# ishika28/Beyond-Binary-Fake-User-Detection-A-Credibility-Aware-Graph-based-Recommender-System

Measured on NVIDIA B200. Metric: edges/sec (3-layer cred-weighted LightGCN fwd+bwd), higher is better.
Workload: dtype f32

## Files before the change

### beyond-binary-fake-user-detection-a-credibility-aware-graph-based-recommender-system_b200/_lib.py

```python
from __future__ import annotations

import ctypes as C
import os
import pathlib
import subprocess

import torch

PKG_DIR = pathlib.Path(__file__).resolve().parent
LIB_PATH = PKG_DIR / "libcredgcn.so"
CSRC_DIR = PKG_DIR / "csrc"

VARIANTS = {"cu": 0, "v2": 1, "da": 2}
ORDERS = {"jacobi": 0, "gs": 1}
PRECISIONS = {"fp32": 0, "bf16x3": 1, "bf16": 2}
OPTIONS = {"L2_TABLE_BYTES": 0, "SPARSE_FIRST_ADJOINT": 1, "PDL": 2, "P2P_ONESHOT_MAX": 3, "P2P_TIMING": 4,
           "P2P_TIMEOUT_MS": 5, "EVAL_DEBUG": 6, "HOT_ROWS": 7, "EVAL_GROUPS": 8}
LONG_ROW = 256
CHUNK = 256


class CgxError(RuntimeError):
    pass

# ... 24 lines not shown
    "cgx_graph_build_workspace_bytes": (C.c_size_t, [C.c_int64, C.c_int32, C.c_int32]),
    "cgx_graph_build": (C.c_int, [_P, _P, C.c_int64, C.c_int32, C.c_int32, _P, C.c_int, _P, _P, _P, _P, _P, _P,
                                  _P, _P, _P, _P, _P, _P, _P, _P, _P, C.c_int, _P, C.c_size_t, _P]),
    "cgx_user_csr": (C.c_int, [_P, _P, C.c_int64, C.c_int32, C.c_int32, _P, _P, _P, C.c_size_t, _P]),
    "cgx_row_schedule_workspace_bytes": (C.c_size_t, [C.c_int32]),
    "cgx_row_schedule": (C.c_int, [_P, C.c_int32, _P, C.POINTER(C.c_int32), C.POINTER(C.c_int32),
                                   C.POINTER(C.c_int32), _P, C.c_size_t, _P]),
    "cgx_row_schedule_chunks": (C.c_int, [C.c_int32, C.c_int32, C.c_int32, _P, _P, _P, C.c_size_t, _P]),
    "cgx_row_schedule_work": (C.c_int, [_P, _P, C.c_int32, C.c_int32, C.c_int32, _P, _P, _P, _P]),
    "cgx_spmm_workspace_bytes": (C.c_size_t, [_CSR, C.c_int32]),
    "cgx_spmm": (C.c_int, [_CSR, C.c_int, C.c_int32, _P, _P, _P, _P, C.c_float, _P, C.c_size_t, _P]),
    "cgx_spmm_sparse_rows": (C.c_int, [_CSR, C.c_int, C.c_int32, _P, _P, _P, _P, _P, C.c_float, _P, C.c_size_t, _P]),
    "cgx_row_flags": (C.c_int, [_P, C.c_int64, C.c_int32, _P, _P]),
    "cgx_spmm_ex": (C.c_int, [_CSR, C.c_int, C.c_int32, _P, _P, _P, _P, _P, _P, C.c_float, _P, C.c_size_t, _P]),
    "cgx_spmm_set_l2_table_bytes": (C.c_int64, [C.c_int64]),
    "cgx_propagate_workspace_bytes": (C.c_size_t, [_CSR, _CSR, C.c_int32]),
    "cgx_propagate_workspace_bytes_for": (C.c_size_t, [_CSR, _CSR, C.c_int32, C.c_int]),
    "cgx_propagate_fwd": (C.c_int, [_CSR, _CSR, C.c_int, C.c_int32, C.c_int32, _P, _P, _P, _P, _P,
                                    C.c_size_t, _P]),
    "cgx_propagate_bwd": (C.c_int, [_CSR, _CSR, C.c_int, C.c_int32, C.c_int32, _P, _P, _P, _P, _P,
                                    C.c_size_t, _P]),
    "cgx_propagate_bwd_flagged": (C.c_int, [_CSR, _CSR, C.c_int, C.c_int32, C.c_int32, _P, _P, _P, _P, _P, _P, _P,
                                            C.c_size_t, _P]),
    "cgx_bpr_mark_rows": (C.c_int, [_P, C.c_int64, C.c_int32, _P, _P, _P]),
    "cgx_bpr_clear_rows": (C.c_int, [_P, C.c_int64, C.c_int32, C.c_int32, _P, _P, _P, _P, _P]),
    "cgx_bpr_workspace_bytes": (C.c_size_t, [C.c_int64, C.c_int32, C.c_int32]),
    "cgx_bpr_plan_workspace_bytes": (C.c_size_t, [C.c_int64]),
    "cgx_bpr_plan": (C.c_int, [_P, _P, _P, C.c_int64, C.c_int32, C.c_int32, _P, _P, C.c_size_t, _P]),
    "cgx_bpr_fwd_bwd": (C.c_int, [_P, _P, _P, C.c_int64, C.c_int64, _P, C.c_int32, C.c_int32, C.c_int32, _P, _P, _P,
                                  _P, _P,
                                  C.c_float, C.c_float, _P, _P, _P, _P, _P, _P, C.c_size_t, _P]),
    "cgx_bpr_apply_ego": (C.c_int, [_P, _P, C.c_int64, C.c_int32, C.c_int32, _P, _P, _P, _P, _P]),
    "cgx_sampler_build_workspace_bytes": (C.c_size_t, [C.c_int32]),
    "cgx_sampler_build": (C.c_int, [_P, C.c_int32, C.c_double, _P, _P, _P, _P, _P, _P, C.c_size_t, _P]),
    "cgx_sample_triples": (C.c_int, [_P, C.c_int64, _P, _P, C.c_int32, _P, _P, _P, _P, _P, C.c_float,
                                     C.c_int32, C.c_uint64, C.c_uint64, _P, _P, _P, _P]),
    "cgx_tick": (C.c_int, [_P, _P]),
    "cgx_adam_step": (C.c_int, [_P, _P, _P, _P, C.c_int64, _P, _P, _P, _P, C.c_int64, C.c_float, C.c_float,
                                C.c_float, C.c_float, _P, C.c_int64, _P]),
    "cgx_comm_alloc": (C.c_int, [C.c_size_t, C.POINTER(C.c_void_p)]),
    "cgx_comm_free": (C.c_int, [_P]),
    "cgx_comm_ipc_handle": (C.c_int, [_P, _P]),
    "cgx_comm_ipc_open": (C.c_int, [_P, C.POINTER(C.c_void_p)]),
    "cgx_comm_ipc_close": (C.c_int, [_P]),
    "cgx_comm_allreduce": (C.c_int, [C.c_int, C.c_int, C.POINTER(C.c_void_p), C.c_size_t, C.c_size_t, C.c_size_t,
                                     C.c_int64, _P, _P]),
# ... 88 lines not shown
```

### beyond-binary-fake-user-detection-a-credibility-aware-graph-based-recommender-system_b200/csrc/spmm.cu

```cuda
#include "common.cuh"

namespace cgx {

constexpr int SP_THREADS = 256;

__device__ __forceinline__ void fma4(float4& a, float v, const float4& x) {
  a.x = fmaf(v, x.x, a.x);
  a.y = fmaf(v, x.y, a.y);
  a.z = fmaf(v, x.z, a.z);
  a.w = fmaf(v, x.w, a.w);
}
__device__ __forceinline__ float4 add4(const float4& a, const float4& b) {
  return make_float4(a.x + b.x, a.y + b.y, a.z + b.z, a.w + b.w);
}
__device__ __forceinline__ float4 scale4(const float4& a, float s) {
  return make_float4(a.x * s, a.y * s, a.z * s, a.w * s);
}

enum { POL_NORMAL = 0, POL_FIRST = 1, POL_LAST = 2 };
template <int POL>
__device__ __forceinline__ void ld256(const float4* p, float4& a, float4& b) {
  if (POL == POL_LAST) {
    asm volatile("ld.global.nc.L1::no_allocate.L2::evict_last.v8.f32 {%0,%1,%2,%3,%4,%5,%6,%7}, [%8];"
                 : "=f"(a.x), "=f"(a.y), "=f"(a.z), "=f"(a.w), "=f"(b.x), "=f"(b.y), "=f"(b.z), "=f"(b.w)
// ... 164 lines not shown
    if constexpr (V == 2) st256<POL>(ACC_OUT + o, a[0], a[1]);
    else {
#pragma unroll
      for (int v = 0; v < V; ++v) ACC_OUT[o + v] = a[v];
    }
  }
}

struct SpmmSched {
  const int32_t* perm;
  const int32_t* chunk_ptr;
  int32_t* arrive;
  int32_t n_chunks, n_huge;
};

template <int G, int V, int UNR, int MINB, bool NZ, bool PUSH, bool HOT>
__global__ void __launch_bounds__(SP_THREADS, MINB) k_spmm(const int32_t* __restrict__ idx,
                                                           const float* __restrict__ val, int64_t n_items,
                                                           SpmmSched sc, const float4* __restrict__ X,
                                                           float4* __restrict__ Y, const float4* ACC_IN,
                                                           float4* ACC_OUT, float acc_scale, float4* partial,
                                                           const uint8_t* __restrict__ nz,
                                                           const uint8_t* __restrict__ acc_nz,
                                                           const int4* __restrict__ work, const SpmmPush ps_in) {
  const SpmmPush ps = PUSH ? ps_in : SpmmPush{0ull, 0, 0};
  constexpr int ROW4 = G * V;
  asm volatile("griddepcontrol.launch_dependents;");
  const int lane = threadIdx.x & (G - 1);
  const uint32_t item = (blockIdx.x * uint32_t(SP_THREADS) + threadIdx.x) / G;
  const unsigned mask = group_mask<G>();
  float4 acc[V];
#pragma unroll
  for (int v = 0; v < V; ++v) acc[v] = make_float4(0.f, 0.f, 0.f, 0.f);
  if (item >= n_items) return;
  const int4 wd = __ldg(work + item);
  const int64_t begin = (int64_t(wd.y) << 32) | uint32_t(wd.x);
  idx += begin;
  val += begin;
  int32_t cf = 0;
  float wf = 0.f;
  if (lane < wd.z) {
    cf = ld_idx<HOT>(idx + lane);
    wf = ld_val<HOT>(val + lane);
  }
  asm volatile("griddepcontrol.wait;" ::: "memory");
  gather_batches<G, V, UNR, NZ, HOT>(idx, val, wd.z, X, lane, mask, cf, wf, acc, nz);
  if (item >= sc.n_chunks) {
    epilogue<G, V, HOT>(wd.w, lane, acc, Y, ACC_IN, ACC_OUT, acc_scale, acc_nz, ps);
    return;
  }
  const int32_t k = wd.w;
#pragma unroll
  for (int v = 0; v < V; ++v) __stcg(partial + int64_t(item) * ROW4 + lane * V + v, acc[v]);
  if (k < sc.n_huge) return;
  const int32_t c0 = __ldg(sc.chunk_ptr + k), c1 = __ldg(sc.chunk_ptr + k + 1);
  __threadfence();
  __syncwarp(mask);
  int prev = 0;
  if (lane == 0) prev = atomicAdd(sc.arrive + k, 1);
  prev = __shfl_sync(mask, prev, 0, G);
  if (prev != c1 - c0 - 1) return;
  __threadfence();
#pragma unroll
  for (int v = 0; v < V; ++v) acc[v] = make_float4(0.f, 0.f, 0.f, 0.f);
  for (int c = c0; c < c1; ++c) {
#pragma unroll
    for (int v = 0; v < V; ++v) acc[v] = add4(acc[v], __ldcg(partial + int64_t(c) * ROW4 + lane * V + v));
  }
  epilogue<G, V, HOT>(int64_t(__ldg(sc.perm + k)), lane, acc, Y, ACC_IN, ACC_OUT, acc_scale, acc_nz, ps);
  if (lane == 0) sc.arrive[k] = 0;
}

template <int G, int V>
__global__ void __launch_bounds__(SP_THREADS) k_spmm_finish(SpmmSched sc, const float4* __restrict__ partial,
                                                            float4* __restrict__ Y, const float4* ACC_IN,
                                                            float4* ACC_OUT, float acc_scale,
                                                            const uint8_t* __restrict__ acc_nz, const SpmmPush ps) {
  constexpr int GROUPS = SP_THREADS / G;
  constexpr int ROW4 = G * V;
  __shared__ float4 red[GROUPS][ROW4];
  const int k = blockIdx.x;
  const int lane = threadIdx.x & (G - 1), grp = threadIdx.x / G;
  const int c0 = __ldg(sc.chunk_ptr + k), c1 = __ldg(sc.chunk_ptr + k + 1);
  float4 acc[V];
#pragma unroll
  for (int v = 0; v < V; ++v) acc[v] = make_float4(0.f, 0.f, 0.f, 0.f);
  for (int c = c0 + grp; c < c1; c += GROUPS) {
#pragma unroll
    for (int v = 0; v < V; ++v) acc[v] = add4(acc[v], __ldg(partial + int64_t(c) * ROW4 + lane * V + v));
  }
#pragma unroll
  for (int v = 0; v < V; ++v) red[grp][lane * V + v] = acc[v];
  __syncthreads();
  if (grp == 0) {
#pragma unroll
    for (int v = 0; v < V; ++v) {
      float4 s = red[0][lane * V + v];
      for (int g = 1; g < GROUPS; ++g) s = add4(s, red[g][lane * V + v]);
      acc[v] = s;
    }
    epilogue<G, V, false>(int64_t(__ldg(sc.perm + k)), lane, acc, Y, ACC_IN, ACC_OUT, acc_scale, acc_nz, ps);
  }
}

// ... 1 lines not shown
  int64_t p = int64_t(blockIdx.x) * blockDim.x + threadIdx.x;
  if (p < n4) out[p] = scale4(in[p], s);
}

__global__ void k_row_flags(const uint4* __restrict__ X, int64_t n4, int32_t row4, uint8_t* __restrict__ flags) {
  const int64_t p = int64_t(blockIdx.x) * blockDim.x + threadIdx.x;
  if (p >= n4) return;
  const uint4 v = X[p];
  if ((v.x | v.y | v.z | v.w) & 0x7fffffffu) flags[p / row4] = 1;
}

static int row_flags(const float* X, int64_t n_rows, int32_t d, uint8_t* flags, cudaStream_t stream) {
  CGX_CUDA(cudaMemsetAsync(flags, 0, size_t(n_rows), stream));
  const int64_t n4 = n_rows * d / 4;
  if (n4 == 0) return CGX_OK;
  k_row_flags<<<(unsigned)ceil_div(n4, 256), 256, 0, stream>>>(reinterpret_cast<const uint4*>(X), n4, d / 4, flags);
  CGX_LAUNCH_CHECK();
  return CGX_OK;
}

template <int G, int V, int UNR, int MINB, bool NZ, bool PUSH, bool HOT>
static int launch_spmm(const cgx_csr* m, const float* val, const float* X, float* Y, const float* ACC_IN,
                       float* ACC_OUT, float acc_scale, void* workspace, size_t workspace_bytes,
                       cudaStream_t stream, const uint8_t* nz, const uint8_t* acc_nz, const SpmmPush ps) {
  constexpr int GROUPS = SP_THREADS / G;
  float4* partial = nullptr;
  if (m->n_long > 0) {
    size_t need = size_t(m->n_chunks) * G * V * sizeof(float4);
    CGX_REQUIRE(workspace != nullptr && workspace_bytes >= need, CGX_ERR_WORKSPACE,
                "spmm: workspace too small for %d long-row chunks", m->n_chunks);
    partial = static_cast<float4*>(workspace);
  }
  SpmmSched sc{m->perm, m->chunk_ptr, m->arrive, m->n_chunks, m->n_huge};
  const int64_t items = int64_t(m->n_chunks) + (m->n_rows - m->n_long);
  cudaLaunchConfig_t cfg = {};
  cfg.gridDim = dim3((unsigned)ceil_div(items, GROUPS));
  cfg.blockDim = dim3(SP_THREADS);
  cfg.dynamicSmemBytes = 0;
  cfg.stream = stream;
  cudaLaunchAttribute attr[1];
  attr[0].id = cudaLaunchAttributeProgrammaticStreamSerialization;
  attr[0].val.programmaticStreamSerializationAllowed = option(CGX_OPT_PDL) != 0 ? 1 : 0;
  cfg.attrs = attr;
  cfg.numAttrs = 1;
  CGX_CUDA(cudaLaunchKernelEx(&cfg, k_spmm<G, V, UNR, MINB, NZ, PUSH, HOT>, HOT ? m->idx_hint : m->idx, val, items, sc,
                              reinterpret_cast<const float4*>(X), reinterpret_cast<float4*>(Y),
                              reinterpret_cast<const float4*>(ACC_IN), reinterpret_cast<float4*>(ACC_OUT), acc_scale,
                              partial, nz, acc_nz, static_cast<const int4*>(m->work), ps));
  CGX_LAUNCH_CHECK();
  if (m->n_huge > 0) {
    k_spmm_finish<G, V><<<(unsigned)m->n_huge, SP_THREADS, 0, stream>>>(
        sc, partial, reinterpret_cast<float4*>(Y), reinterpret_cast<const float4*>(ACC_IN),
        reinterpret_cast<float4*>(ACC_OUT), acc_scale, acc_nz, ps);
    CGX_LAUNCH_CHECK();
  }
  return CGX_OK;
}

#define CGX_SPMM_ARGS m, val, X, Y, ACC_IN, ACC_OUT, acc_scale, ws, ws_bytes, stream, nz, acc_nz, ps

template <int G, int V, int UNR>
static int spmm_flavour(const cgx_csr* m, const float* val, const float* X, float* Y, const float* ACC_IN,
                        float* ACC_OUT, float acc_scale, void* ws, size_t ws_bytes, cudaStream_t stream,
                        const uint8_t* nz, const uint8_t* acc_nz, const SpmmPush ps, bool hot) {
  const bool push = ps.rows_per > 0;
  if constexpr (V == 2) {
    if (hot && nz == nullptr) {
      if (push) return launch_spmm<G, V, UNR, 4, false, true, true>(CGX_SPMM_ARGS);
      return launch_spmm<G, V, UNR, 4, false, false, true>(CGX_SPMM_ARGS);
    }
  }
  if (push) {
    if (nz) return launch_spmm<G, V, UNR, 4, true, true, false>(CGX_SPMM_ARGS);
    return launch_spmm<G, V, UNR, 4, false, true, false>(CGX_SPMM_ARGS);
  }
  if (nz) return launch_spmm<G, V, UNR, 4, true, false, false>(CGX_SPMM_ARGS);
  return launch_spmm<G, V, UNR, 4, false, false, false>(CGX_SPMM_ARGS);
}

#define CGX_FLAVOUR_ARGS m, val, X, Y, ACC_IN, ACC_OUT, acc_scale, ws, ws_bytes, stream, nz, acc_nz, ps, hot

static int spmm_dispatch(const cgx_csr* m, int use_bwd, int32_t d, const float* X, float* Y, const float* ACC_IN,
                         float* ACC_OUT, float acc_scale, void* ws, size_t ws_bytes, cudaStream_t stream,
                         const uint8_t* nz = nullptr, const SpmmPush ps = SpmmPush{0ull, 0, 0},
                         const uint8_t* acc_nz = nullptr) {
  CGX_REQUIRE(m && m->perm && m->work && (m->nnz == 0 || (m->idx && m->val_fwd && m->val_bwd)) && X, CGX_ERR_ARG,
              "spmm: NULL pointer (cgx_csr needs idx, both value arrays and the cgx_row_schedule* outputs)");
  CGX_REQUIRE(m->n_long == 0 || (m->chunk_ptr && m->arrive), CGX_ERR_ARG, "spmm: chunk tables missing");
  CGX_REQUIRE(Y || ACC_OUT || ps.rows_per > 0, CGX_ERR_ARG, "spmm: no output requested");
  const float* val = use_bwd ? m->val_bwd : m->val_fwd;
  if (m->n_rows == 0) return CGX_OK;
  const bool beyond_l2 = int64_t(m->n_cols) * int64_t(d) * 4 > option(CGX_OPT_L2_TABLE_BYTES);
  const bool hot = beyond_l2 && m->idx_hint != nullptr && option(CGX_OPT_HOT_ROWS) != 0;
  switch (d) {
    case 16: return spmm_flavour<4, 1, 4>(CGX_FLAVOUR_ARGS);
    case 32: return spmm_flavour<8, 1, 8>(CGX_FLAVOUR_ARGS);
    case 64:
      if (beyond_l2) return spmm_flavour<8, 2, 4>(CGX_FLAVOUR_ARGS);
      return spmm_flavour<16, 1, 8>(CGX_FLAVOUR_ARGS);
    case 128:
      if (beyond_l2) return spmm_flavour<16, 2, 4>(CGX_FLAVOUR_ARGS);
      return spmm_flavour<32, 1, 8>(CGX_FLAVOUR_ARGS);
    case 256: return spmm_flavour<32, 2, 4>(CGX_FLAVOUR_ARGS);
    default:
      set_error("spmm: emb_dim %d unsupported (16, 32, 64, 128, 256)", d);
      return CGX_ERR_UNSUPPORTED;
  }
}

__global__ void k_hot_flags(const int32_t* __restrict__ col_by_degree, int32_t n_hot, uint8_t* __restrict__ hot) {
  const int32_t k = blockIdx.x * blockDim.x + threadIdx.x;
  if (k < n_hot) hot[__ldg(col_by_degree + k)] = 1;
// ... 68 lines not shown

extern "C" int cgx_spmm_set_push_peers(void* const* peer_bases, int world) {
  CGX_REQUIRE(peer_bases != nullptr && world >= 1 && world <= 16, CGX_ERR_ARG, "spmm_set_push_peers: bad argument");
  char* h[16] = {nullptr};
  for (int p = 0; p < world; ++p) h[p] = static_cast<char*>(peer_bases[p]);
  CGX_CUDA(cudaMemcpyToSymbol(c_push_base, h, sizeof(h)));
  return CGX_OK;
}

extern "C" int cgx_spmm_push(const cgx_csr* m, int use_bwd_values, int32_t d, const float* X,
                             const uint8_t* x_row_nonzero, size_t stage_off, int rank, int world, int32_t rows_per,
                             void* workspace, size_t workspace_bytes, void* stream) {
  CGX_REQUIRE(m != nullptr && world >= 1 && world <= 16 && rank >= 0 && rank < world && rows_per > 0 &&
                  int64_t(rows_per) * world >= m->n_rows && stage_off % 16 == 0,
              CGX_ERR_ARG, "spmm_push: bad rank / world / rows_per");
  const SpmmPush ps{(unsigned long long)stage_off, rows_per, rank};
  return spmm_dispatch(m, use_bwd_values, d, X, nullptr, nullptr, nullptr, 1.0f, workspace, workspace_bytes,
                       static_cast<cudaStream_t>(stream), x_row_nonzero, ps);
}

extern "C" int cgx_row_flags(const float* X, int64_t n_rows, int32_t d, uint8_t* flags, void* stream) {
  CGX_REQUIRE(X && flags && n_rows >= 0 && d > 0 && d % 4 == 0, CGX_ERR_ARG, "row_flags: bad argument");
  return row_flags(X, n_rows, d, flags, static_cast<cudaStream_t>(stream));
}

static size_t propagate_ws(const cgx_csr* by_user, const cgx_csr* by_item, int32_t d, int n_buf) {
  if (!by_user || !by_item) return 0;
  size_t long_ws = spmm_ws(by_user, d) > spmm_ws(by_item, d) ? spmm_ws(by_user, d) : spmm_ws(by_item, d);
  return n_buf * (align_up(size_t(by_user->n_rows) * d * 4) + align_up(size_t(by_item->n_rows) * d * 4)) + long_ws +
         align_up(size_t(by_user->n_rows)) + align_up(size_t(by_item->n_rows)) + 256;
}

extern "C" size_t cgx_propagate_workspace_bytes(const cgx_csr* by_user, const cgx_csr* by_item, int32_t d) {
  return propagate_ws(by_user, by_item, d, 2);
}

extern "C" size_t cgx_propagate_workspace_bytes_for(const cgx_csr* by_user, const cgx_csr* by_item, int32_t d,
                                                    int order) {
  return propagate_ws(by_user, by_item, d, order == CGX_ORDER_GS ? 1 : 2);
}

extern "C" int cgx_propagate_fwd(const cgx_csr* by_user, const cgx_csr* by_item, int order, int32_t K, int32_t d,
                                 const float* e0_u, const float* e0_i, float* out_u, float* out_i,
                                 void* workspace, size_t workspace_bytes, void* stream_) {
  cudaStream_t stream = static_cast<cudaStream_t>(stream_);
  CGX_REQUIRE(by_user && by_item && e0_u && e0_i && out_u && out_i, CGX_ERR_ARG, "propagate_fwd: NULL pointer");
// ... 33 lines not shown
    ci = ni;
  }
  return CGX_OK;
}

__global__ void k_scale_rows(const float4* __restrict__ in, const uint8_t* __restrict__ nz, float4* __restrict__ out,
                             int64_t n_rows, int32_t row4, float s) {
  const int64_t r = (int64_t(blockIdx.x) * blockDim.x + threadIdx.x) / 32;
  if (r >= n_rows || __ldg(nz + r) == 0) return;
  for (int p = threadIdx.x & 31; p < row4; p += 32) out[r * row4 + p] = scale4(in[r * row4 + p], s);
}

extern "C" int cgx_propagate_bwd(const cgx_csr* by_user, const cgx_csr* by_item, int order, int32_t K, int32_t d,
                                 const float* g_u, const float* g_i, float* d_e0_u, float* d_e0_i,
                                 void* workspace, size_t workspace_bytes, void* stream_) {
  return cgx_propagate_bwd_flagged(by_user, by_item, order, K, d, g_u, g_i, nullptr, nullptr, d_e0_u, d_e0_i, workspace,
                                   workspace_bytes, stream_);
}

extern "C" int cgx_propagate_bwd_flagged(const cgx_csr* by_user, const cgx_csr* by_item, int order, int32_t K,
                                         int32_t d, const float* g_u, const float* g_i, const uint8_t* g_u_rows,
                                         const uint8_t* g_i_rows, float* d_e0_u, float* d_e0_i, void* workspace,
                                         size_t workspace_bytes, void* stream_) {
  cudaStream_t stream = static_cast<cudaStream_t>(stream_);
  CGX_REQUIRE((g_u_rows == nullptr) == (g_i_rows == nullptr), CGX_ERR_ARG,
              "propagate_bwd_flagged: pass both row-flag arrays or neither");
  CGX_REQUIRE(by_user && by_item && g_u && g_i && d_e0_u && d_e0_i, CGX_ERR_ARG, "propagate_bwd: NULL pointer");
  CGX_REQUIRE(K >= 1, CGX_ERR_ARG, "propagate_bwd: num_layers must be >= 1");
  CGX_REQUIRE(order == CGX_ORDER_JACOBI || order == CGX_ORDER_GS, CGX_ERR_ARG, "propagate_bwd: bad order");
  CGX_REQUIRE(workspace_bytes >= cgx_propagate_workspace_bytes_for(by_user, by_item, d, order), CGX_ERR_WORKSPACE,
              "propagate_bwd: workspace too small");
  const int64_t U = by_user->n_rows, I = by_item->n_rows;
  Arena ws(workspace, workspace_bytes);
  const bool one = order == CGX_ORDER_GS;
  float* ub[2];
  float* ib[2];
  ub[0] = ws.take<float>(U * d);
  ub[1] = one ? ub[0] : ws.take<float>(U * d);
  ib[0] = ws.take<float>(I * d);
  ib[1] = one ? ib[0] : ws.take<float>(I * d);
  size_t lws = spmm_ws(by_user, d) > spmm_ws(by_item, d) ? spmm_ws(by_user, d) : spmm_ws(by_item, d);
  void* lw = ws.take<char>(lws);
  CGX_REQUIRE(ws.ok, CGX_ERR_WORKSPACE, "propagate_bwd: workspace too small");
  const float s = 1.0f / float(K + 1);
  const bool given = g_u_rows != nullptr;
  const bool sparse = given || option(CGX_OPT_SPARSE_FIRST_ADJOINT) != 0;
  uint8_t* nz_u = given ? const_cast<uint8_t*>(g_u_rows) : ws.take<uint8_t>(U);
  uint8_t* nz_i = given ? const_cast<uint8_t*>(g_i_rows) : ws.take<uint8_t>(I);
  CGX_REQUIRE(ws.ok, CGX_ERR_WORKSPACE, "propagate_bwd: workspace too small");
  if (order == CGX_ORDER_JACOBI) {
    const float* bu = g_u;
    const float* bi = g_i;
    if (sparse && !given) {
      CGX_TRY(row_flags(g_u, U, d, nz_u, stream));
      CGX_TRY(row_flags(g_i, I, d, nz_i, stream));
    }
    for (int k = 0; k < K; ++k) {
      const bool last = k == K - 1;
      float* nu = last ? d_e0_u : ub[k & 1];
      float* ni = last ? d_e0_i : ib[k & 1];
      const float sc = last ? s : 1.0f;
      const bool sp = sparse && k == 0;
      const SpmmPush nops{0ull, 0, 0};
      CGX_TRY(spmm_dispatch(by_user, 1, d, bi, nullptr, g_u, nu, sc, lw, lws, stream, sp ? nz_i : nullptr, nops,
                            sparse ? nz_u : nullptr));
      CGX_TRY(spmm_dispatch(by_item, 1, d, bu, nullptr, g_i, ni, sc, lw, lws, stream, sp ? nz_u : nullptr, nops,
                            sparse ? nz_i : nullptr));
      bu = nu;
      bi = ni;
    }
  } else {
    const float* bu = g_u;
    if (sparse && !given) {
      CGX_TRY(row_flags(g_u, U, d, nz_u, stream));
      CGX_TRY(row_flags(g_i, I, d, nz_i, stream));
    }
    const SpmmPush nops{0ull, 0, 0};
    for (int k = 0; k < K; ++k) {
      const bool last = k == K - 1;
      float* ni = ib[0];
      float* nu = last ? d_e0_u : ub[k & 1];
      CGX_TRY(spmm_dispatch(by_item, 1, d, bu, nullptr, g_i, ni, 1.0f, lw, lws, stream,
                            sparse && k == 0 ? nz_u : nullptr, nops, sparse ? nz_i : nullptr));
      CGX_TRY(spmm_dispatch(by_user, 1, d, ni, nullptr, g_u, nu, last ? s : 1.0f, lw, lws, stream, nullptr, nops,
                            sparse ? nz_u : nullptr));
      bu = nu;
    }
    const int64_t n4 = I * d / 4;
    if (given) {
      CGX_CUDA(cudaMemsetAsync(d_e0_i, 0, size_t(I) * d * 4, stream));
      if (I > 0) {
        k_scale_rows<<<(unsigned)ceil_div(I * 32, 256), 256, 0, stream>>>(
            reinterpret_cast<const float4*>(g_i), nz_i, reinterpret_cast<float4*>(d_e0_i), I, d / 4, s);
        CGX_LAUNCH_CHECK();
      }
    } else {
      k_scale<<<(unsigned)ceil_div(n4, 256), 256, 0, stream>>>(reinterpret_cast<const float4*>(g_i),
                                                               reinterpret_cast<float4*>(d_e0_i), n4, s);
      CGX_LAUNCH_CHECK();
    }
  }
  return CGX_OK;
}
```

### beyond-binary-fake-user-detection-a-credibility-aware-graph-based-recommender-system_b200/model.py

```python
from __future__ import annotations

import torch

from . import _lib
from ._lib import check, lib, ptr, stream_ptr, workspace
from .graph import CredGraph, graph_of


def _f32c(t: torch.Tensor) -> torch.Tensor:
    if t.dtype != torch.float32:
        raise _lib.CgxError(f"credgcn kernels are fp32, got {t.dtype}")
    return t.contiguous()


def _i64c(t, device) -> torch.Tensor:
    return torch.as_tensor(t, device=device).to(torch.int64).contiguous()


def propagate_forward(graph: CredGraph, e0_u, e0_i, num_layers: int, order: str):
    e0_u, e0_i = _f32c(e0_u), _f32c(e0_i)
    d = e0_u.shape[1]
    out_u, out_i = torch.empty_like(e0_u), torch.empty_like(e0_i)
    ws = graph.propagate_workspace(d, order)
    with torch.cuda.device(graph.device):
# ... 37 lines not shown
def spmm_sparse_rows(csr, x, flags=None, use_bwd_values=False):
    x = _f32c(x)
    flags = row_flags(x) if flags is None else flags
    d = x.shape[1]
    y = torch.empty(csr.n_rows, d, dtype=torch.float32, device=x.device)
    ws = workspace(lib().cgx_spmm_workspace_bytes(csr.ref(), d), x.device)
    with torch.cuda.device(x.device):
        check(lib().cgx_spmm_sparse_rows(csr.ref(), int(use_bwd_values), d, ptr(x), ptr(flags), ptr(y), None, None,
                                         1.0, ptr(ws), ws.numel(), stream_ptr(x.device)))
    return y


def bpr_plan(graph: CredGraph, users, pos, neg, plan=None):
    dev = graph.device
    users, pos, neg = _i64c(users, dev), _i64c(pos, dev), _i64c(neg, dev)
    B = users.numel()
    if plan is None:
        plan = torch.empty(3 * B, dtype=torch.int64, device=dev)
    ws = workspace(lib().cgx_bpr_plan_workspace_bytes(B), dev)
    with torch.cuda.device(dev):
        check(lib().cgx_bpr_plan(ptr(users), ptr(pos), ptr(neg), B, graph.num_users, graph.num_items, ptr(plan),
                                 ptr(ws), ws.numel(), stream_ptr(dev)))
    return plan


def bpr_fused(graph: CredGraph, f_u, f_i, e0_u, e0_i, users, pos, neg, reg_weight, fair_weight=0.0, pop=None,
              g_u=None, g_i=None, plan=None, bufs=None, batch_total=0):
    dev = f_u.device
    f_u, f_i, e0_u, e0_i = _f32c(f_u), _f32c(f_i), _f32c(e0_u), _f32c(e0_i)
    users, pos, neg = _i64c(users, dev), _i64c(pos, dev), _i64c(neg, dev)
    B, d = users.numel(), f_u.shape[1]
    if plan is None:
        plan = bpr_plan(graph, users, pos, neg)
    if g_u is None:
        g_u = torch.zeros_like(f_u)
    if g_i is None:
        g_i = torch.zeros_like(f_i)
    if bufs is None:
        bufs = bpr_buffers(graph, B, dev)
    loss, ego_rows, ego_coef, ws = bufs
    pop_t = None if pop is None else _f32c(torch.as_tensor(pop, device=dev))
    with torch.cuda.device(dev):
        check(lib().cgx_bpr_fwd_bwd(ptr(users), ptr(pos), ptr(neg), B, int(batch_total), ptr(plan), graph.num_users,
                                    graph.num_items,
                                    d, ptr(f_u), ptr(f_i), ptr(e0_u), ptr(e0_i), ptr(pop_t), float(reg_weight),
                                    float(fair_weight), ptr(loss), ptr(g_u), ptr(g_i), ptr(ego_rows),
# ... 181 lines not shown
            check(lib().cgx_tick(ptr(self.step_dev), st))
            check(lib().cgx_adam_step(ptr(pu.data), ptr(_f32c(pu.grad)), ptr(self.m[0]), ptr(self.v[0]), pu.numel(),
                                      ptr(pi.data), ptr(_f32c(pi.grad)), ptr(self.m[1]), ptr(self.v[1]), pi.numel(),
                                      self.lr, self.betas[0], self.betas[1], self.eps, ptr(self.step_dev), 0, st))

    def state_dict(self):
        return {"step": int(self.step_dev.item()), "exp_avg": self.m, "exp_avg_sq": self.v, "lr": self.lr,
                "betas": self.betas, "eps": self.eps}


class TrainStep:

    def __init__(self, model: _Base, lr=1e-3, reg_weight=1e-4, fair_weight=0.0, pop=None, optimizer=None,
                 sampler=None):
        self.model, self.graph = model, model.graph
        self.reg, self.fair = float(reg_weight), float(fair_weight)
        dev = model.user_emb.weight.device
        self.pop = None if pop is None else torch.as_tensor(pop, dtype=torch.float32, device=dev).contiguous()
        eu, ei = model.user_emb.weight, model.item_emb.weight
        self.f_u, self.f_i = torch.empty_like(eu), torch.empty_like(ei)
        self.g_u, self.g_i = torch.zeros_like(eu), torch.zeros_like(ei)
        self.nz_u = torch.zeros(eu.shape[0], dtype=torch.uint8, device=dev)
        self.nz_i = torch.zeros(ei.shape[0], dtype=torch.uint8, device=dev)
        eu.grad, ei.grad = torch.empty_like(eu), torch.empty_like(ei)
        self.opt = optimizer or FusedAdam(eu, ei, lr=lr)
        self.sampler = sampler
        self.phase_events = None
        self.side = torch.cuda.Stream(device=dev)
        self.tick = torch.zeros(1, dtype=torch.int64, device=dev)
        self._bufs = {}
        self._graph = None

    def _mark(self, marks):
        if self.phase_events is not None:
            ev = torch.cuda.Event(enable_timing=True)
            ev.record(torch.cuda.current_stream(self.graph.device))
            marks.append(ev)

    def _batch_bufs(self, B, dev):
        if B not in self._bufs:
            self._bufs[B] = (torch.empty(3 * B, dtype=torch.int64, device=dev), bpr_buffers(self.graph, B, dev))
        return self._bufs[B]

    @torch.no_grad()
    def forward_backward(self, users, pos, neg):
        m, g = self.model, self.graph
        eu, ei = m.user_emb.weight, m.item_emb.weight
        d, K, order = eu.shape[1], m.num_layers, _lib.ORDERS[m.ORDER]
        ws = g.propagate_workspace(d, order)
        dev = eu.device
        users, pos, neg = _i64c(users, dev), _i64c(pos, dev), _i64c(neg, dev)
        plan, bufs = self._batch_bufs(users.numel(), dev)
        marks = []
        with torch.cuda.device(dev):
            main = torch.cuda.current_stream(dev)
            self._mark(marks)
            self.side.wait_stream(main)
            with torch.cuda.stream(self.side):
                bpr_plan(g, users, pos, neg, plan)
            st = stream_ptr(dev)
            check(lib().cgx_propagate_fwd(g.by_user.ref(), g.by_item.ref(), order, K, d, ptr(eu), ptr(ei),
                                          ptr(self.f_u), ptr(self.f_i), ptr(ws), ws.numel(), st))
            self._mark(marks)
            main.wait_stream(self.side)
            loss, _, _, ego_rows, ego_coef = bpr_fused(g, self.f_u, self.f_i, eu, ei, users, pos, neg, self.reg,
                                                       self.fair, self.pop, self.g_u, self.g_i, plan, bufs)
            n_ent = ego_rows.numel()
            check(lib().cgx_bpr_mark_rows(ptr(ego_rows), n_ent, g.num_users, ptr(self.nz_u), ptr(self.nz_i), st))
            self._mark(marks)
            check(lib().cgx_propagate_bwd_flagged(g.by_user.ref(), g.by_item.ref(), order, K, d, ptr(self.g_u),
                                                  ptr(self.g_i), ptr(self.nz_u), ptr(self.nz_i), ptr(eu.grad),
                                                  ptr(ei.grad), ptr(ws), ws.numel(), st))
            self._mark(marks)
            apply_ego(g, ego_rows, ego_coef, eu, ei, eu.grad, ei.grad)
            check(lib().cgx_bpr_clear_rows(ptr(ego_rows), n_ent, g.num_users, d, ptr(self.g_u), ptr(self.g_i),
                                           ptr(self.nz_u), ptr(self.nz_i), st))
        if self.phase_events is not None:
            self.phase_events.append(marks)
        return loss

    def __call__(self, users, pos, neg):
        loss = self.forward_backward(users, pos, neg)
        self.opt.step()
        return loss

    @torch.no_grad()
    def _sampled_step(self, users):
        dev = self.graph.device
        with torch.cuda.device(dev):
            check(lib().cgx_tick(ptr(self.tick), stream_ptr(dev)))
        pos, neg = self.sampler.sample(users, offset=0, offset_dev=self.tick)
        return self.__call__(users, pos, neg)

    def capture(self, batch: int, preserve_state: bool = True):
        if self.sampler is None:
# ... 42 lines not shown
```

### include/credgcn.h

```cpp
#ifndef CREDGCN_H_
#define CREDGCN_H_

#include <stddef.h>
#include <stdint.h>

#if defined(__GNUC__)
#pragma GCC visibility push(default)
#endif

#ifdef __cplusplus
extern "C" {
#endif

typedef enum {
  CGX_OK = 0,
  CGX_ERR_ARG = -1,
  CGX_ERR_WORKSPACE = -2,
  CGX_ERR_CUDA = -3,
  CGX_ERR_UNSUPPORTED = -4
} cgx_status;

typedef enum { CGX_VARIANT_CU = 0, CGX_VARIANT_V2 = 1, CGX_VARIANT_DA = 2 } cgx_variant;
typedef enum { CGX_ORDER_JACOBI = 0, CGX_ORDER_GS = 1 } cgx_order;
typedef enum { CGX_SCORE_FP32 = 0, CGX_SCORE_BF16X3 = 1, CGX_SCORE_BF16 = 2 } cgx_score_precision;
// ... 81 lines not shown
                         const uint8_t* x_row_nonzero, float* Y, const float* ACC_IN, float* ACC_OUT,
                         float acc_scale, void* workspace, size_t workspace_bytes, void* stream);
int cgx_row_flags(const float* X, int64_t n_rows, int32_t d, uint8_t* flags, void* stream);
int cgx_spmm_ex(const cgx_csr* m, int use_bwd_values, int32_t d, const float* X, const uint8_t* x_row_nonzero,
                float* Y, const float* ACC_IN, const uint8_t* acc_row_nonzero, float* ACC_OUT, float acc_scale,
                void* workspace, size_t workspace_bytes, void* stream);

int64_t cgx_spmm_set_l2_table_bytes(int64_t bytes);

size_t cgx_propagate_workspace_bytes(const cgx_csr* by_user, const cgx_csr* by_item, int32_t d);
size_t cgx_propagate_workspace_bytes_for(const cgx_csr* by_user, const cgx_csr* by_item, int32_t d, int order);

int cgx_propagate_fwd(const cgx_csr* by_user, const cgx_csr* by_item, int order, int32_t num_layers,
                      int32_t d, const float* e0_u, const float* e0_i, float* out_u, float* out_i,
                      void* workspace, size_t workspace_bytes, void* stream);

int cgx_propagate_bwd(const cgx_csr* by_user, const cgx_csr* by_item, int order, int32_t num_layers,
                      int32_t d, const float* g_u, const float* g_i, float* d_e0_u, float* d_e0_i,
                      void* workspace, size_t workspace_bytes, void* stream);
int cgx_propagate_bwd_flagged(const cgx_csr* by_user, const cgx_csr* by_item, int order, int32_t num_layers,
                              int32_t d, const float* g_u, const float* g_i, const uint8_t* g_u_rows,
                              const uint8_t* g_i_rows, float* d_e0_u, float* d_e0_i, void* workspace,
                              size_t workspace_bytes, void* stream);

size_t cgx_bpr_plan_workspace_bytes(int64_t batch);
int cgx_bpr_plan(const int64_t* users, const int64_t* pos, const int64_t* neg, int64_t batch,
                 int32_t num_users, int32_t num_items, uint64_t* plan,
                 void* workspace, size_t workspace_bytes, void* stream);
size_t cgx_bpr_workspace_bytes(int64_t batch, int32_t num_users, int32_t num_items);
int cgx_bpr_fwd_bwd(const int64_t* users, const int64_t* pos, const int64_t* neg, int64_t batch,
                    int64_t batch_total, const uint64_t* plan, int32_t num_users, int32_t num_items, int32_t d,
                    const float* f_u, const float* f_i, const float* e0_u, const float* e0_i,
                    const float* pop, float reg_weight, float fair_weight,
                    float* loss_out, float* g_u, float* g_i,
                    int32_t* ego_rows, float* ego_coef,
                    void* workspace, size_t workspace_bytes, void* stream);
int cgx_bpr_apply_ego(const int32_t* ego_rows, const float* ego_coef, int64_t n_entries,
                      int32_t num_users, int32_t d, const float* e0_u, const float* e0_i,
                      float* d_e0_u, float* d_e0_i, void* stream);
int cgx_bpr_mark_rows(const int32_t* ego_rows, int64_t n_entries, int32_t num_users, uint8_t* nz_u, uint8_t* nz_i,
                      void* stream);
int cgx_bpr_clear_rows(const int32_t* ego_rows, int64_t n_entries, int32_t num_users, int32_t d, float* g_u,
                       float* g_i, uint8_t* nz_u, uint8_t* nz_i, void* stream);

size_t cgx_sampler_build_workspace_bytes(int32_t num_items);
int cgx_sampler_build(const int32_t* deg_i, int32_t num_items, double gamma,
// ... 76 lines not shown
```

Measured before the change: 1.238 billion.

## Restrict first backward adjoint layer to the batch's item frontier

Adds a batch-frontier kernel that flags the positive and negative items of the batch plus every item adjacent to a batch user. The backward propagation then uses these flags as an output-row mask on the item SpMM at layer 0 and as gather flags on the following user SpMM, so rows outside the frontier are skipped. The goal is to cut gather traffic when the item table does not fit in L2. Risk: correctness rests on the frontier being a superset of the rows whose gradients are nonzero, and the flag computation adds an extra launch on a side stream.

Measured after the change: 1.284 billion (median of 6 runs). +3.7%, better.

```diff
diff --git a/beyond-binary-fake-user-detection-a-credibility-aware-graph-based-recommender-system_b200/_lib.py b/beyond-binary-fake-user-detection-a-credibility-aware-graph-based-recommender-system_b200/_lib.py
--- a/beyond-binary-fake-user-detection-a-credibility-aware-graph-based-recommender-system_b200/_lib.py
+++ b/beyond-binary-fake-user-detection-a-credibility-aware-graph-based-recommender-system_b200/_lib.py
@@ -70,6 +70,9 @@
                                     C.c_size_t, _P]),
     "cgx_propagate_bwd_flagged": (C.c_int, [_CSR, _CSR, C.c_int, C.c_int32, C.c_int32, _P, _P, _P, _P, _P, _P, _P,
                                             C.c_size_t, _P]),
+    "cgx_propagate_bwd_frontier": (C.c_int, [_CSR, _CSR, C.c_int, C.c_int32, C.c_int32, _P, _P, _P, _P, _P, _P,
+                                             _P, _P, C.c_size_t, _P]),
+    "cgx_batch_frontier": (C.c_int, [_CSR, _P, _P, _P, C.c_int64, _P, _P]),
     "cgx_bpr_mark_rows": (C.c_int, [_P, C.c_int64, C.c_int32, _P, _P, _P]),
     "cgx_bpr_clear_rows": (C.c_int, [_P, C.c_int64, C.c_int32, C.c_int32, _P, _P, _P, _P, _P]),
     "cgx_bpr_workspace_bytes": (C.c_size_t, [C.c_int64, C.c_int32, C.c_int32]),
diff --git a/beyond-binary-fake-user-detection-a-credibility-aware-graph-based-recommender-system_b200/csrc/spmm.cu b/beyond-binary-fake-user-detection-a-credibility-aware-graph-based-recommender-system_b200/csrc/spmm.cu
--- a/beyond-binary-fake-user-detection-a-credibility-aware-graph-based-recommender-system_b200/csrc/spmm.cu
+++ b/beyond-binary-fake-user-detection-a-credibility-aware-graph-based-recommender-system_b200/csrc/spmm.cu
@@ -210,6 +210,7 @@
                                                            float4* ACC_OUT, float acc_scale, float4* partial,
                                                            const uint8_t* __restrict__ nz,
                                                            const uint8_t* __restrict__ acc_nz,
+                                                           const uint8_t* __restrict__ out_rows,
                                                            const int4* __restrict__ work, const SpmmPush ps_in) {
   const SpmmPush ps = PUSH ? ps_in : SpmmPush{0ull, 0, 0};
   constexpr int ROW4 = G * V;
@@ -232,6 +233,9 @@
     wf = ld_val<HOT>(val + lane);
   }
   asm volatile("griddepcontrol.wait;" ::: "memory");
+  if (NZ && !PUSH && out_rows != nullptr &&
+      __ldg(out_rows + (item >= sc.n_chunks ? wd.w : __ldg(sc.perm + wd.w))) == 0)
+    return;
   gather_batches<G, V, UNR, NZ, HOT>(idx, val, wd.z, X, lane, mask, cf, wf, acc, nz);
   if (item >= sc.n_chunks) {
     epilogue<G, V, HOT>(wd.w, lane, acc, Y, ACC_IN, ACC_OUT, acc_scale, acc_nz, ps);
@@ -263,11 +267,13 @@
 __global__ void __launch_bounds__(SP_THREADS) k_spmm_finish(SpmmSched sc, const float4* __restrict__ partial,
                                                             float4* __restrict__ Y, const float4* ACC_IN,
                                                             float4* ACC_OUT, float acc_scale,
-                                                            const uint8_t* __restrict__ acc_nz, const SpmmPush ps) {
+                                                            const uint8_t* __restrict__ acc_nz,
+                                                            const uint8_t* __restrict__ out_rows, const SpmmPush ps) {
   constexpr int GROUPS = SP_THREADS / G;
   constexpr int ROW4 = G * V;
   __shared__ float4 red[GROUPS][ROW4];
   const int k = blockIdx.x;
+  if (out_rows != nullptr && __ldg(out_rows + __ldg(sc.perm + k)) == 0) return;
   const int lane = threadIdx.x & (G - 1), grp = threadIdx.x / G;
   const int c0 = __ldg(sc.chunk_ptr + k), c1 = __ldg(sc.chunk_ptr + k + 1);
   float4 acc[V];
@@ -315,7 +321,8 @@
 template <int G, int V, int UNR, int MINB, bool NZ, bool PUSH, bool HOT>
 static int launch_spmm(const cgx_csr* m, const float* val, const float* X, float* Y, const float* ACC_IN,
                        float* ACC_OUT, float acc_scale, void* workspace, size_t workspace_bytes,
-                       cudaStream_t stream, const uint8_t* nz, const uint8_t* acc_nz, const SpmmPush ps) {
+                       cudaStream_t stream, const uint8_t* nz, const uint8_t* acc_nz, const uint8_t* out_rows,
+                       const SpmmPush ps) {
   constexpr int GROUPS = SP_THREADS / G;
   float4* partial = nullptr;
   if (m->n_long > 0) {
@@ -339,23 +346,24 @@
   CGX_CUDA(cudaLaunchKernelEx(&cfg, k_spmm<G, V, UNR, MINB, NZ, PUSH, HOT>, HOT ? m->idx_hint : m->idx, val, items, sc,
                               reinterpret_cast<const float4*>(X), reinterpret_cast<float4*>(Y),
                               reinterpret_cast<const float4*>(ACC_IN), reinterpret_cast<float4*>(ACC_OUT), acc_scale,
-                              partial, nz, acc_nz, static_cast<const int4*>(m->work), ps));
+                              partial, nz, acc_nz, out_rows, static_cast<const int4*>(m->work), ps));
   CGX_LAUNCH_CHECK();
   if (m->n_huge > 0) {
     k_spmm_finish<G, V><<<(unsigned)m->n_huge, SP_THREADS, 0, stream>>>(
         sc, partial, reinterpret_cast<float4*>(Y), reinterpret_cast<const float4*>(ACC_IN),
-        reinterpret_cast<float4*>(ACC_OUT), acc_scale, acc_nz, ps);
+        reinterpret_cast<float4*>(ACC_OUT), acc_scale, acc_nz, out_rows, ps);
     CGX_LAUNCH_CHECK();
   }
   return CGX_OK;
 }
 
-#define CGX_SPMM_ARGS m, val, X, Y, ACC_IN, ACC_OUT, acc_scale, ws, ws_bytes, stream, nz, acc_nz, ps
+#define CGX_SPMM_ARGS m, val, X, Y, ACC_IN, ACC_OUT, acc_scale, ws, ws_bytes, stream, nz, acc_nz, out_rows, ps
 
 template <int G, int V, int UNR>
 static int spmm_flavour(const cgx_csr* m, const float* val, const float* X, float* Y, const float* ACC_IN,
                         float* ACC_OUT, float acc_scale, void* ws, size_t ws_bytes, cudaStream_t stream,
-                        const uint8_t* nz, const uint8_t* acc_nz, const SpmmPush ps, bool hot) {
+                        const uint8_t* nz, const uint8_t* acc_nz, const uint8_t* out_rows, const SpmmPush ps,
+                        bool hot) {
   const bool push = ps.rows_per > 0;
   if constexpr (V == 2) {
     if (hot && nz == nullptr) {
@@ -371,16 +379,18 @@
   return launch_spmm<G, V, UNR, 4, false, false, false>(CGX_SPMM_ARGS);
 }
 
-#define CGX_FLAVOUR_ARGS m, val, X, Y, ACC_IN, ACC_OUT, acc_scale, ws, ws_bytes, stream, nz, acc_nz, ps, hot
+#define CGX_FLAVOUR_ARGS m, val, X, Y, ACC_IN, ACC_OUT, acc_scale, ws, ws_bytes, stream, nz, acc_nz, out_rows, ps, hot
 
 static int spmm_dispatch(const cgx_csr* m, int use_bwd, int32_t d, const float* X, float* Y, const float* ACC_IN,
                          float* ACC_OUT, float acc_scale, void* ws, size_t ws_bytes, cudaStream_t stream,
                          const uint8_t* nz = nullptr, const SpmmPush ps = SpmmPush{0ull, 0, 0},
-                         const uint8_t* acc_nz = nullptr) {
+                         const uint8_t* acc_nz = nullptr, const uint8_t* out_rows = nullptr) {
   CGX_REQUIRE(m && m->perm && m->work && (m->nnz == 0 || (m->idx && m->val_fwd && m->val_bwd)) && X, CGX_ERR_ARG,
               "spmm: NULL pointer (cgx_csr needs idx, both value arrays and the cgx_row_schedule* outputs)");
   CGX_REQUIRE(m->n_long == 0 || (m->chunk_ptr && m->arrive), CGX_ERR_ARG, "spmm: chunk tables missing");
   CGX_REQUIRE(Y || ACC_OUT || ps.rows_per > 0, CGX_ERR_ARG, "spmm: no output requested");
+  CGX_REQUIRE(out_rows == nullptr || (nz != nullptr && ps.rows_per == 0), CGX_ERR_ARG,
+              "spmm: an output-row mask needs gather flags and no push mode");
   const float* val = use_bwd ? m->val_bwd : m->val_fwd;
   if (m->n_rows == 0) return CGX_OK;
   const bool beyond_l2 = int64_t(m->n_cols) * int64_t(d) * 4 > option(CGX_OPT_L2_TABLE_BYTES);
@@ -495,6 +505,37 @@
 extern "C" int cgx_row_flags(const float* X, int64_t n_rows, int32_t d, uint8_t* flags, void* stream) {
   CGX_REQUIRE(X && flags && n_rows >= 0 && d > 0 && d % 4 == 0, CGX_ERR_ARG, "row_flags: bad argument");
   return row_flags(X, n_rows, d, flags, static_cast<cudaStream_t>(stream));
+}
+
+__device__ __forceinline__ int64_t clamp_row(int64_t x, int64_t n) { return (x < 0 || x >= n) ? 0 : x; }
+__global__ void k_batch_frontier(const int64_t* __restrict__ indptr, const int32_t* __restrict__ idx,
+                                 const int64_t* __restrict__ users, const int64_t* __restrict__ pos,
+                                 const int64_t* __restrict__ neg, int64_t B, int32_t U, int32_t I,
+                                 uint8_t* __restrict__ flags) {
+  const int64_t t = (int64_t(blockIdx.x) * blockDim.x + threadIdx.x) / 32;
+  const int lane = threadIdx.x & 31;
+  if (t >= B) return;
+  if (lane == 0) {
+    flags[clamp_row(pos[t], I)] = 1;
+    flags[clamp_row(neg[t], I)] = 1;
+  }
+  const int64_t u = clamp_row(users[t], U);
+  const int64_t end = indptr[u + 1];
+  for (int64_t j = indptr[u] + lane; j < end; j += 32) flags[idx[j]] = 1;
+}
+
+extern "C" int cgx_batch_frontier(const cgx_csr* by_user, const int64_t* users, const int64_t* pos,
+                                  const int64_t* neg, int64_t B, uint8_t* flags_i, void* stream_) {
+  cudaStream_t stream = static_cast<cudaStream_t>(stream_);
+  CGX_REQUIRE(by_user && by_user->indptr && (by_user->nnz == 0 || by_user->idx) && users && pos && neg && flags_i,
+              CGX_ERR_ARG, "batch_frontier: NULL pointer");
+  CGX_REQUIRE(B > 0 && B < (int64_t(1) << 29) && by_user->n_rows > 0 && by_user->n_cols > 0, CGX_ERR_ARG,
+              "batch_frontier: bad batch size %lld or empty graph", (long long)B);
+  CGX_CUDA(cudaMemsetAsync(flags_i, 0, size_t(by_user->n_cols), stream));
+  k_batch_frontier<<<(unsigned)ceil_div(B * 32, 256), 256, 0, stream>>>(
+      by_user->indptr, by_user->idx, users, pos, neg, B, by_user->n_rows, by_user->n_cols, flags_i);
+  CGX_LAUNCH_CHECK();
+  return CGX_OK;
 }
 
 static size_t propagate_ws(const cgx_csr* by_user, const cgx_csr* by_item, int32_t d, int n_buf) {
@@ -574,6 +615,14 @@
                                          int32_t d, const float* g_u, const float* g_i, const uint8_t* g_u_rows,
                                          const uint8_t* g_i_rows, float* d_e0_u, float* d_e0_i, void* workspace,
                                          size_t workspace_bytes, void* stream_) {
+  return cgx_propagate_bwd_frontier(by_user, by_item, order, K, d, g_u, g_i, g_u_rows, g_i_rows, nullptr, d_e0_u,
+                                    d_e0_i, workspace, workspace_bytes, stream_);
+}
+
+extern "C" int cgx_propagate_bwd_frontier(const cgx_csr* by_user, const cgx_csr* by_item, int order, int32_t K,
+                                          int32_t d, const float* g_u, const float* g_i, const uint8_t* g_u_rows,
+                                          const uint8_t* g_i_rows, const uint8_t* front_i, float* d_e0_u,
+                                          float* d_e0_i, void* workspace, size_t workspace_bytes, void* stream_) {
   cudaStream_t stream = static_cast<cudaStream_t>(stream_);
   CGX_REQUIRE((g_u_rows == nullptr) == (g_i_rows == nullptr), CGX_ERR_ARG,
               "propagate_bwd_flagged: pass both row-flag arrays or neither");
@@ -600,6 +649,7 @@
   uint8_t* nz_u = given ? const_cast<uint8_t*>(g_u_rows) : ws.take<uint8_t>(U);
   uint8_t* nz_i = given ? const_cast<uint8_t*>(g_i_rows) : ws.take<uint8_t>(I);
   CGX_REQUIRE(ws.ok, CGX_ERR_WORKSPACE, "propagate_bwd: workspace too small");
+  const uint8_t* front = sparse ? front_i : nullptr;
   if (order == CGX_ORDER_JACOBI) {
     const float* bu = g_u;
     const float* bi = g_i;
@@ -614,10 +664,11 @@
       const float sc = last ? s : 1.0f;
       const bool sp = sparse && k == 0;
       const SpmmPush nops{0ull, 0, 0};
-      CGX_TRY(spmm_dispatch(by_user, 1, d, bi, nullptr, g_u, nu, sc, lw, lws, stream, sp ? nz_i : nullptr, nops,
+      const uint8_t* bi_nz = sp ? nz_i : (k == 1 ? front : nullptr);
+      CGX_TRY(spmm_dispatch(by_user, 1, d, bi, nullptr, g_u, nu, sc, lw, lws, stream, bi_nz, nops,
                             sparse ? nz_u : nullptr));
       CGX_TRY(spmm_dispatch(by_item, 1, d, bu, nullptr, g_i, ni, sc, lw, lws, stream, sp ? nz_u : nullptr, nops,
-                            sparse ? nz_i : nullptr));
+                            sparse ? nz_i : nullptr, k == 0 && !last ? front : nullptr));
       bu = nu;
       bi = ni;
     }
@@ -632,9 +683,10 @@
       const bool last = k == K - 1;
       float* ni = ib[0];
       float* nu = last ? d_e0_u : ub[k & 1];
+      const uint8_t* f0 = k == 0 ? front : nullptr;
       CGX_TRY(spmm_dispatch(by_item, 1, d, bu, nullptr, g_i, ni, 1.0f, lw, lws, stream,
-                            sparse && k == 0 ? nz_u : nullptr, nops, sparse ? nz_i : nullptr));
-      CGX_TRY(spmm_dispatch(by_user, 1, d, ni, nullptr, g_u, nu, last ? s : 1.0f, lw, lws, stream, nullptr, nops,
+                            sparse && k == 0 ? nz_u : nullptr, nops, sparse ? nz_i : nullptr, f0));
+      CGX_TRY(spmm_dispatch(by_user, 1, d, ni, nullptr, g_u, nu, last ? s : 1.0f, lw, lws, stream, f0, nops,
                             sparse ? nz_u : nullptr));
       bu = nu;
     }
diff --git a/beyond-binary-fake-user-detection-a-credibility-aware-graph-based-recommender-system_b200/model.py b/beyond-binary-fake-user-detection-a-credibility-aware-graph-based-recommender-system_b200/model.py
--- a/beyond-binary-fake-user-detection-a-credibility-aware-graph-based-recommender-system_b200/model.py
+++ b/beyond-binary-fake-user-detection-a-credibility-aware-graph-based-recommender-system_b200/model.py
@@ -83,6 +83,17 @@
         check(lib().cgx_bpr_plan(ptr(users), ptr(pos), ptr(neg), B, graph.num_users, graph.num_items, ptr(plan),
                                  ptr(ws), ws.numel(), stream_ptr(dev)))
     return plan
+
+
+def batch_frontier(graph: CredGraph, users, pos, neg, flags=None):
+    dev = graph.device
+    users, pos, neg = _i64c(users, dev), _i64c(pos, dev), _i64c(neg, dev)
+    if flags is None:
+        flags = torch.empty(graph.num_items, dtype=torch.uint8, device=dev)
+    with torch.cuda.device(dev):
+        check(lib().cgx_batch_frontier(graph.by_user.ref(), ptr(users), ptr(pos), ptr(neg), users.numel(), ptr(flags),
+                                       stream_ptr(dev)))
+    return flags
 
 
 def bpr_fused(graph: CredGraph, f_u, f_i, e0_u, e0_i, users, pos, neg, reg_weight, fair_weight=0.0, pop=None,
@@ -310,6 +321,7 @@
         self.g_u, self.g_i = torch.zeros_like(eu), torch.zeros_like(ei)
         self.nz_u = torch.zeros(eu.shape[0], dtype=torch.uint8, device=dev)
         self.nz_i = torch.zeros(ei.shape[0], dtype=torch.uint8, device=dev)
+        self.front_i = torch.zeros(ei.shape[0], dtype=torch.uint8, device=dev)
         eu.grad, ei.grad = torch.empty_like(eu), torch.empty_like(ei)
         self.opt = optimizer or FusedAdam(eu, ei, lr=lr)
         self.sampler = sampler
@@ -339,6 +351,7 @@
         dev = eu.device
         users, pos, neg = _i64c(users, dev), _i64c(pos, dev), _i64c(neg, dev)
         plan, bufs = self._batch_bufs(users.numel(), dev)
+        front = self.front_i if g.num_items * d * 4 > _lib.get_option("L2_TABLE_BYTES") else None
         marks = []
         with torch.cuda.device(dev):
             main = torch.cuda.current_stream(dev)
@@ -346,6 +359,8 @@
             self.side.wait_stream(main)
             with torch.cuda.stream(self.side):
                 bpr_plan(g, users, pos, neg, plan)
+                if front is not None:
+                    batch_frontier(g, users, pos, neg, front)
             st = stream_ptr(dev)
             check(lib().cgx_propagate_fwd(g.by_user.ref(), g.by_item.ref(), order, K, d, ptr(eu), ptr(ei),
                                           ptr(self.f_u), ptr(self.f_i), ptr(ws), ws.numel(), st))
@@ -356,9 +371,9 @@
             n_ent = ego_rows.numel()
             check(lib().cgx_bpr_mark_rows(ptr(ego_rows), n_ent, g.num_users, ptr(self.nz_u), ptr(self.nz_i), st))
             self._mark(marks)
-            check(lib().cgx_propagate_bwd_flagged(g.by_user.ref(), g.by_item.ref(), order, K, d, ptr(self.g_u),
-                                                  ptr(self.g_i), ptr(self.nz_u), ptr(self.nz_i), ptr(eu.grad),
-                                                  ptr(ei.grad), ptr(ws), ws.numel(), st))
+            check(lib().cgx_propagate_bwd_frontier(g.by_user.ref(), g.by_item.ref(), order, K, d, ptr(self.g_u),
+                                                   ptr(self.g_i), ptr(self.nz_u), ptr(self.nz_i), ptr(front),
+                                                   ptr(eu.grad), ptr(ei.grad), ptr(ws), ws.numel(), st))
             self._mark(marks)
             apply_ego(g, ego_rows, ego_coef, eu, ei, eu.grad, ei.grad)
             check(lib().cgx_bpr_clear_rows(ptr(ego_rows), n_ent, g.num_users, d, ptr(self.g_u), ptr(self.g_i),
diff --git a/include/credgcn.h b/include/credgcn.h
--- a/include/credgcn.h
+++ b/include/credgcn.h
@@ -127,6 +127,12 @@
                               int32_t d, const float* g_u, const float* g_i, const uint8_t* g_u_rows,
                               const uint8_t* g_i_rows, float* d_e0_u, float* d_e0_i, void* workspace,
                               size_t workspace_bytes, void* stream);
+int cgx_propagate_bwd_frontier(const cgx_csr* by_user, const cgx_csr* by_item, int order, int32_t num_layers,
+                               int32_t d, const float* g_u, const float* g_i, const uint8_t* g_u_rows,
+                               const uint8_t* g_i_rows, const uint8_t* front_i, float* d_e0_u, float* d_e0_i,
+                               void* workspace, size_t workspace_bytes, void* stream);
+int cgx_batch_frontier(const cgx_csr* by_user, const int64_t* users, const int64_t* pos, const int64_t* neg,
+                       int64_t batch, uint8_t* flags_i, void* stream);
 
 size_t cgx_bpr_plan_workspace_bytes(int64_t batch);
 int cgx_bpr_plan(const int64_t* users, const int64_t* pos, const int64_t* neg, int64_t batch,
diff --git a/profiles/frontier.py b/profiles/frontier.py
--- /dev/null
+++ b/profiles/frontier.py
@@ -0,0 +1,137 @@
+import argparse
+import json
+import pathlib
+import sys
+
+HERE = pathlib.Path(__file__).resolve().parent
+BATCH = 4096
+
+
+def c4_setup(tree, with_step):
+    sys.path.insert(0, str(tree))
+    import numpy as np
+    import torch
+    from credgcn import graph, model, sampler, synth
+    dev = torch.device("cuda")
+    shp = synth.SHAPES["C4"]
+    sg = synth.make_graph_device("C4", dev)
+    U, I = sg.num_users, sg.num_items
+    gr = graph.build_graph(sg.train_edges, U, I, sg.cred, shp["variant"], dev)
+    sg.train_edges = sg.val_edges = sg.test_edges = None
+    torch.cuda.empty_cache()
+    torch.manual_seed(42)
+    samp = sampler.TripleSampler(gr, 0.7, 0.75, 50, seed=42)
+    train_users = torch.nonzero(gr.deg_u > 0).reshape(-1).cpu().numpy()
+    np.random.default_rng(42).shuffle(train_users)
+    n_batches = min(max(len(train_users) // BATCH, 1), 64)
+    batches = [torch.from_numpy(train_users[s * BATCH:(s + 1) * BATCH]).to(dev) for s in range(n_batches)]
+    step = None
+    if with_step:
+        net = model.LightGCN(U, I, shp["emb_dim"], shp["num_layers"], gr.operator("A"), gr.operator("C")).to(dev)
+        step = model.TrainStep(net, lr=1e-3, reg_weight=1e-4, sampler=samp)
+    return dict(torch=torch, np=np, model=model, gr=gr, samp=samp, batches=batches, shp=shp, step=step)
+
+
+def stats(args):
+    e = c4_setup(HERE.parent, False)
+    torch, model, gr = e["torch"], e["model"], e["gr"]
+    d = e["shp"]["emb_dim"]
+    deg_i = (gr.by_item.indptr[1:] - gr.by_item.indptr[:-1]).to(torch.int64)
+    n_hot = min((48 << 20) // (4 * d), gr.num_items)
+    hot = torch.zeros(gr.num_items, dtype=torch.bool, device=deg_i.device)
+    hot[gr.by_item.perm[:n_hot].long()] = True
+    rows = []
+    for s, users in enumerate(e["batches"][:args.batches]):
+        pos, neg = e["samp"].sample(users, offset=s)
+        f = model.batch_frontier(gr, users, pos, neg).bool()
+        rows.append(dict(batch=s, front_items=int(f.sum()), front_edges=int(deg_i[f].sum()),
+                         front_edges_hot=int(deg_i[f & hot].sum())))
+    mean = {k: sum(r[k] for r in rows) / len(rows) for k in rows[0] if k != "batch"}
+    by_user, by_item = gr.by_user, gr.by_item
+    out = dict(workload="C4", batch_users=BATCH, emb_dim=d, num_users=gr.num_users, num_items=gr.num_items,
+               nnz=int(gr.nnz), item_rows_long=by_item.n_long, item_chunks=by_item.n_chunks,
+               user_rows_long=by_user.n_long, user_chunks=by_user.n_chunks, hot_item_rows=n_hot,
+               gpu=torch.cuda.get_device_name(), mean=mean, batches=rows)
+    pathlib.Path(args.out).write_text(json.dumps(out, indent=1))
+    print(json.dumps(dict(mean=mean, nnz=out["nnz"], items=out["num_items"])))
+
+
+def kernels(args):
+    e = c4_setup(pathlib.Path(args.tree).resolve(), True)
+    torch, step, batches = e["torch"], e["step"], e["batches"]
+    for s in range(3):
+        step.step(batches[s])
+    torch.cuda.synchronize()
+    steps = []
+    with torch.profiler.profile(activities=[torch.profiler.ProfilerActivity.CUDA]) as prof:
+        for s in range(3, 3 + args.steps):
+            step.step(batches[s])
+            torch.cuda.synchronize()
+    ev = sorted((k for k in prof.events() if k.device_type == torch.autograd.DeviceType.CUDA),
+                key=lambda k: k.time_range.start)
+    spmm = [k for k in ev if "k_spmm" in k.name]
+    per = len(spmm) // args.steps
+    for s in range(args.steps):
+        steps.append([dict(kernel=k.name.split("(")[0].replace("void ", "").replace("cgx::", ""),
+                           ms=round(k.time_range.elapsed_us() / 1e3, 3)) for k in spmm[s * per:(s + 1) * per]])
+    other = [dict(kernel=k.name.split("(")[0].replace("void ", "").replace("cgx::", ""),
+                  ms=round(k.time_range.elapsed_us() / 1e3, 3)) for k in ev if "frontier" in k.name]
+    out = dict(tree=str(args.tree), gpu=torch.cuda.get_device_name(), spmm_launches_per_step=per, steps=steps,
+               frontier_launches=other)
+    pathlib.Path(args.out).write_text(json.dumps(out, indent=1))
+    for s in steps:
+        print(" ".join(f"{l['ms']:.2f}" for l in s))
+
+
+def traffic(args):
+    st = json.loads(pathlib.Path(args.stats).read_text())
+    m, d, B = st["mean"], st["emb_dim"], st["batch_users"]
+    U, I, E = st["num_users"], st["num_items"], st["nnz"]
+    row = 4 * d
+    out_items = I - m["front_items"]
+    l7 = (16 * (st["item_chunks"] + I - st["item_rows_long"]) + 8 * m["front_edges"] + 64 * out_items
+          + row * m["front_items"] + row * B + row * 2 * B + I + U)
+    l8 = (16 * (st["user_chunks"] + U - st["user_rows_long"]) + 8 * E + row * U + row * m["front_items"]
+          + row * B + I + U)
+    path = HERE / "r2_traffic.json"
+    data = json.loads(path.read_text())
+    c4 = data["C4"]
+    src = f"profiles/{pathlib.Path(args.stats).name} (frontier.py traffic)"
+    for i, gb, kind in ((6, l7, "item rows masked by the batch's item frontier F"),
+                        (7, l8, "user rows gathering only the rows of F")):
+        old = c4["launches"][i]
+        c4["launches"][i] = dict(kernel=old.get("captured_kernel", old["kernel"]), gb=round(gb / 1e9, 3),
+                                 computed=True, what=kind, source=src,
+                                 captured_before_frontier=dict(ms=old.get("ms"), gb=old.get("gb"),
+                                                               l2_hit_pct=old.get("l2_hit_pct"))
+                                 if "captured_before_frontier" not in old else old["captured_before_frontier"])
+    c4["launches"][6]["kernel"] = "k_spmm<16, 2, 4, 4, 1, 0, 0>"
+    c4["launches"][7]["kernel"] = "k_spmm<16, 2, 4, 4, 1, 0, 0>"
+    c4["bytes_per_step"] = sum(l["gb"] for l in c4["launches"]) * 1e9
+    c4["source"] = ("computed: ncu --set full of bench.py's eager step (profiles/r2_ncu_spmm_c4.txt) for launches "
+                    f"1-6 and 9-12, bytes computed from the measured item frontier ({src}) for launches 7 and 8")
+    c4["note"] = ("launches 7 and 8 (the Gauss-Seidel adjoint at k = 0) are computed, not captured: they now touch "
+                  "only the batch's item frontier; their capture before that change is kept under "
+                  "captured_before_frontier")
+    path.write_text(json.dumps(data, indent=1))
+    print(f"launch 7: {l7 / 1e9:.3f} GB, launch 8: {l8 / 1e9:.3f} GB, step: {c4['bytes_per_step'] / 1e9:.1f} GB")
+
+
+def main():
+    ap = argparse.ArgumentParser()
+    sub = ap.add_subparsers(dest="cmd", required=True)
+    a = sub.add_parser("stats")
+    a.add_argument("out")
+    a.add_argument("--batches", type=int, default=16)
+    a = sub.add_parser("kernels")
+    a.add_argument("out")
+    a.add_argument("--tree", default=str(HERE.parent))
+    a.add_argument("--steps", type=int, default=2)
+    a = sub.add_parser("traffic")
+    a.add_argument("stats")
+    args = ap.parse_args()
+    dict(stats=stats, kernels=kernels, traffic=traffic)[args.cmd](args)
+
+
+if __name__ == "__main__":
+    main()
```
